# AE-HYU/monte_carlo_localization

Measured on AMD Instinct MI355X. Metric: MCL updates/sec (particle*beam/s), higher is better.
Workload: dtype f64; 1 GPU; 4194304 particles/GPU x 1081 beams, Spielberg_map (2000x2000 @ 0.05796), initial cloud N((0.0, 0.0, 0.0),(0.5 m,0.5 m,0.4 rad)) (tracking regime), action (0.05, 0.0, 0.01), stock sensor/motion params, multinomial resampling, Philox seed 42; the timed updates follow 5 warm-up updates (the particle set has resampled to motion-noise width); particles_total=4194304, beams=1081, parallelism=single GPU

## Files before the change

monte_carlo_localization_amd/csrc/mcl_engine.hip:

```cpp
#include "../../include/mcl_hip_engine.h"

#include <hip/hip_runtime.h>
#include <hip/hip_ext.h>
#include <rocprim/device/device_radix_sort.hpp>

#include <algorithm>
#include <chrono>
#include <cmath>
#include <cstdio>
#include <cstring>
#include <string>
#include <vector>

#include "mcl_engine_internal.h"
#include "mcl_kernels.h"
#include "mcl_host_math.h"
#include "mcl_lfield.h"

static_assert(MCL_WEDGES == mcl::kWedges || MCL_KWEDGES != 16, "include/mcl_hip_engine.h and csrc/mcl_wedge.h disagree");

using namespace mcl_host;

namespace {

thread_local std::string g_create_error;

int ensure_lt(mcl_engine *h)
{
    size_t need = (size_t)(h->P + 1) * h->bpad;
    if (need > h->lt_capacity) {
        dfree(h->d_Lt);
        HIPCHK(h, hipMalloc(&h->d_Lt, 2 * need * sizeof(float)));
        h->lt_capacity = need;
    }
    h->ltd_cols = (h->B + 2 * h->beam_margin + 64) & ~63;
    const size_t need_d = (size_t)mcl::sweep_table_rows(h->P) * h->ltd_cols;
    if (need_d > h->ltd_capacity) {
        dfree(h->d_Ltd);
        HIPCHK(h, hipMalloc(&h->d_Ltd, need_d * sizeof(double)));
        h->ltd_capacity = need_d;
        h->ltd_ready = false;
    }
    return MCL_OK;
}

void build_ltd(mcl_engine *h);

int weight_stats(mcl_engine *h, bool from_log, const double *d_max_override, bool defer_sums = false)
{
    const int64_t n = h->N;
    const double *src = from_log ? h->d_logw : h->d_w;
    const double *max_parts = nullptr;
    if (!d_max_override) {
        if (!(from_log && h->max_partials_ready))
            hipLaunchKernelGGL(mcl::k_reduce_max, dim3(mcl::kRedBlocks), dim3(mcl::kRedThreads), 0, h->stream, src, n, h->d_maxpart);
        max_parts = h->d_maxpart;
    }
    h->max_partials_ready = false;
    hipLaunchKernelGGL(mcl::k_weights, dim3(mcl::kRedBlocks), dim3(mcl::kRedThreads), 0, h->stream, src, from_log ? 1 : 0,
                       d_max_override ? d_max_override : h->d_scalars, h->d_x[h->cur], h->d_y[h->cur], h->d_th[h->cur], n, h->d_w, h->d_q, h->d_part,
                       (from_log && h->cfg.resample_neff_permille > 0) ? h->d_carry[h->carry_idx ^ 1] : (double *)nullptr,
                       max_parts, mcl::kRedBlocks);
    h->carry_pending = from_log && h->cfg.resample_neff_permille > 0;
    if (!from_log) h->carry_valid = false;
    if (defer_sums) h->sums_pending = true;
    else hipLaunchKernelGGL(mcl::k_final_sums, dim3(1), dim3(mcl::kRedThreads), 0, h->stream, h->d_part, mcl::kRedBlocks, h->d_scalars);
    HIPCHK(h, hipGetLastError());
    return MCL_OK;
}

int fetch_scalars(mcl_engine *h)
{
    HIPCHK(h, hipMemcpyAsync(h->h_result, h->d_result, kResultWords * 8, hipMemcpyDeviceToHost, h->stream));
    HIPCHK(h, hipStreamSynchronize(h->stream));
    unpack_result(h);
    return MCL_OK;
}

bool sweep_hybrid(const mcl_engine *h)
{
    return h->sweep_global && h->env_sweep_hybrid != 0 && h->rec_ok && h->sweep_hyb_layout_ok && h->d_beam_err != nullptr &&
           h->d_distw != nullptr && h->d_distg != nullptr && (size_t)mcl::kSwWinBytes + (size_t)h->ltd_cols * 8 <= 80 * 1024 - 64;
}

bool sweep_far_expected(const mcl_engine *h) { return h->far_fresh || h->h_result[15] >= mcl::kFarWindowedMin / 2; }
bool sweep_hybrid_decide(mcl_engine *h)
{
    if (!sweep_hybrid(h)) return false;
    if (h->env_sweep_hybrid == 2) return true;
    if (h->far_fresh) { h->hyb_backoff = 0; h->hyb_skip = 0; return false; }
    if (h->last_sweep_global == 2) {
        if (h->h_result[15] >= mcl::kFarWindowedMin / 2) { h->hyb_backoff = h->hyb_backoff ? std::min(32, 2 * h->hyb_backoff) : 1; h->hyb_skip = h->hyb_backoff; }
        else h->hyb_backoff = 0;
    }
    if (h->hyb_skip > 0) { --h->hyb_skip; return false; }
// ... 586 lines not shown
}

int mcl_host::fail(mcl_engine *h, int code, const char *msg) { if (h) h->err = msg; return code; }
int mcl_host::fail(mcl_engine *h, int code, const std::string &msg) { return fail(h, code, msg.c_str()); }

std::string &mcl_host::create_error() { return g_create_error; }

bool mcl_host::ready(mcl_engine *h, bool need_particles)
{
    return h && h->have_map && h->B > 0 && (!need_particles || h->have_particles);
}

float mcl_host::elapsed(hipEvent_t a, hipEvent_t b)
{
    float ms = 0.f;
    (void)hipEventElapsedTime(&ms, a, b);
    return ms;
}

void mcl_host::graph_reset(mcl_engine *h)
{
    for (int k = 0; k < 2; ++k)
        if (h->graph_exec[k]) { (void)hipGraphExecDestroy(h->graph_exec[k]); h->graph_exec[k] = nullptr; }
    h->graph_warm = false;
    h->prep_cache_valid = false; h->prep_folded = false;
    h->layout_valid = false; h->layout_stale_used = false; h->keys_done = false;
    h->pc_ready = false;
}

int mcl_host::scan_weights(mcl_engine *h, const uint64_t *d_q, uint64_t *d_cdf, int64_t n, uint64_t offset, uint64_t *d_total)
{
    int nb = (int)((n + mcl::kScanTile - 1) / mcl::kScanTile);
    mcl::CompactOut co{};
    const bool own = d_q == h->d_q && d_cdf == h->d_cdf && offset == 0 && !h->env_no_compact && h->d_ccdf;
    if (own) {
        co.block_cnt = h->d_blockcnt; co.ccdf = h->d_ccdf; co.cidx = h->d_cidx; co.crec = h->d_crec; co.ctop = h->d_ctop;
        co.x = h->d_x[h->cur]; co.y = h->d_y[h->cur]; co.th = h->d_th[h->cur];
        co.cap = (uint32_t)h->compact_cap; co.total = h->d_result + 16;
    }
    hipLaunchKernelGGL(mcl::k_scan_partials, dim3(nb), dim3(mcl::kScanThreads), 0, h->stream, d_q, n, h->d_blocktot, co.block_cnt);
    const bool fold = h->sums_pending && d_q == h->d_q;
    hipLaunchKernelGGL(mcl::k_scan_spine, dim3(1), dim3(1024), 0, h->stream, h->d_blocktot, nb, offset, d_total, co.block_cnt, co.total,
                       fold ? h->d_part : (const double *)nullptr, mcl::kRedBlocks, h->d_scalars);
    if (fold) h->sums_pending = false;
    const size_t nlead = (size_t)((n + 15) >> mcl::kLeaderShift) + 1;
    if (nlead > h->leaders_capacity) {
        graph_reset(h);
        dfree(h->d_leaders);
        HIPCHK(h, hipMalloc(&h->d_leaders, nlead * 8));
        h->leaders_capacity = nlead;
    }
    if (h->bind_sensor_event && own && !h->capturing) {
        hipExtLaunchKernelGGL(mcl::k_scan_final, dim3(nb), dim3(mcl::kScanThreads), 0, h->stream, nullptr, h->ev[EV_SENSOR], 0, d_q, n, h->d_blocktot, d_cdf,
                              h->d_leaders, co);
        h->ev_sensor_bound = true; h->bind_sensor_event = false;
    } else {
        hipLaunchKernelGGL(mcl::k_scan_final, dim3(nb), dim3(mcl::kScanThreads), 0, h->stream, d_q, n, h->d_blocktot, d_cdf, h->d_leaders, co);
    }
    HIPCHK(h, hipGetLastError());
    h->blocktot_for = d_cdf; h->blocktot_n = n;
    if (d_cdf == h->d_cdf) { h->compact_n = -1; h->compact_pending = own; h->list_epoch++; }
    return MCL_OK;
}

void mcl_host::unpack_result(mcl_engine *h)
{
    std::memcpy(h->h_scalars, h->h_result, 8 * sizeof(double));
    std::memcpy(h->h_counters, h->h_result + 8, 4 * sizeof(unsigned long long));
    h->h_fix_count = h->h_result[12];
    uint64_t qt;
    std::memcpy(&qt, &h->h_scalars[2], 8);
    h->q_total = qt;
    h->global_sums[0] = h->h_scalars[1];
    h->global_sums[1] = h->h_scalars[3];
    h->global_sums[2] = h->h_scalars[4];
    h->global_sums[3] = h->h_scalars[5];
    h->global_sums[4] = h->h_scalars[6];
    if (h->compact_pending) {
        const unsigned long long na = h->h_result[16];
        h->compact_n = na <= (unsigned long long)h->compact_cap ? (int64_t)na : -1;
        h->compact_pending = false;
    }
}

int mcl_abi_version(void) { return MCL_ABI_VERSION; }

const char *mcl_last_error(const mcl_engine_t *h) { return h ? h->err.c_str() : g_create_error.c_str(); }

int mcl_create(const mcl_config_t *cfg, mcl_engine_t **out)
{
// ... 11 lines not shown
    }
    if (const char *why = bad_sensor_fields(*cfg)) { g_create_error = why; return MCL_ERR_INVALID_ARG; }
    {
        const double disp[3] = {cfg->motion_dispersion_x, cfg->motion_dispersion_y, cfg->motion_dispersion_theta};
        for (double v : disp)
            if (!std::isfinite(v) || v < 0.0) {
                g_create_error = "bad config (motion_dispersion_x/y/theta must be finite and >= 0)";
                return MCL_ERR_INVALID_ARG;
            }
    }
    int ndev = 0;
    if (hipGetDeviceCount(&ndev) != hipSuccess || ndev <= 0 || cfg->device < 0 || cfg->device >= ndev) {
        g_create_error = "no HIP device (this engine has no CPU path)";
        return MCL_ERR_NO_DEVICE;
    }
    hipDeviceProp_t prop;
    if (hipSetDevice(cfg->device) != hipSuccess || hipGetDeviceProperties(&prop, cfg->device) != hipSuccess) {
        g_create_error = "hipSetDevice/hipGetDeviceProperties failed";
        return MCL_ERR_NO_DEVICE;
    }
    if (std::strncmp(prop.gcnArchName, "gfx950", 6) != 0) {
        g_create_error = std::string("device is ") + prop.gcnArchName + ", engine is built for gfx950 only";
        return MCL_ERR_NO_DEVICE;
    }
    mcl_engine *h = new mcl_engine();
    h->cfg = *cfg;
    if (const char *e = getenv("MCL_CELL_MIN")) h->env_cell_min = atoll(e);
    if (const char *e = getenv("MCL_CELL_SLICE")) h->env_cell_slice = atoll(e);
    if (const char *e = getenv("MCL_QSLICES_PER_CU")) h->env_qslices_per_cu = atoi(e);
    if (const char *e = getenv("MCL_QSIDE")) h->env_qside = atoi(e);
    if (const char *e = getenv("MCL_SWEEP_G")) h->env_sweep_g = atoi(e);
    if (const char *e = getenv("MCL_TINY_POLL")) h->env_tiny_poll = atoi(e);
    if (const char *e = getenv("MCL_NO_COMPACT")) h->env_no_compact = atoi(e);
    if (const char *e = getenv("MCL_SORT")) h->env_sort_radix = std::strcmp(e, "radix") == 0 ? 1 : (std::strcmp(e, "hist") == 0 ? 0 : -1);
    if (const char *e = getenv("MCL_DEBUG_WG")) h->env_debug_wg = e;
    h->env_no_bucket_cuts = getenv("MCL_NO_BUCKET_CUTS") != nullptr;
    if (const char *e = getenv("MCL_SWEEP_GLOBAL")) h->env_sweep_global = atoi(e) != 0;
    if (const char *e = getenv("MCL_SWEEP_HYBRID")) h->env_sweep_hybrid = atoi(e);
    if (const char *e = getenv("MCL_SW_GUIDE")) h->env_sw_guide = atoi(e);
    if (const char *e = getenv("MCL_SW_SPLIT16")) h->env_sw_split16 = atoi(e) != 0;
    if (const char *e = getenv("MCL_SWEEP_PAIRS")) h->env_sweep_pairs = atoi(e) != 0 ? 1 : 0;
    h->env_no_obs_overlap = getenv("MCL_NO_OBS_OVERLAP") != nullptr;
    h->env_no_prep_fold = getenv("MCL_NO_PREP_FOLD") != nullptr;
    h->env_no_stale_layout = getenv("MCL_NO_STALE_LAYOUT") != nullptr;
    h->env_comm_no_pregather = getenv("MCL_COMM_NO_PREGATHER") != nullptr;
    h->env_comm_no_lists = getenv("MCL_COMM_NO_LISTS") != nullptr;
    h->num_cu = prop.multiProcessorCount;
    h->cap = cfg->max_particles;
    auto bail = [&](const char *what) {
        g_create_error = std::string(what) + ": " + h->err;
        mcl_destroy(h);
        return MCL_ERR_HIP;
    };
#define CRT(call)                                                         \
    do {                                                                  \
        hipError_t e_ = (call);                                           \
        if (e_ != hipSuccess) { h->err = hipGetErrorString(e_); return bail(#call); } \
    } while (0)
    CRT(hipStreamCreateWithFlags(&h->stream, hipStreamNonBlocking));
    CRT(hipStreamCreateWithFlags(&h->stream2, hipStreamNonBlocking));
    CRT(hipEventCreateWithFlags(&h->ev_obs, hipEventDisableTiming));
    for (int i = 0; i < EV_COUNT; ++i) CRT(hipEventCreate(&h->ev[i]));
    const size_t nb = (size_t)h->cap * sizeof(double);
    for (int b = 0; b < 2; ++b) {
        CRT(hipMalloc(&h->d_x[b], nb)); CRT(hipMalloc(&h->d_y[b], nb)); CRT(hipMalloc(&h->d_th[b], nb));
        CRT(hipMalloc(&h->d_pack[b], (size_t)h->cap * sizeof(double4)));
    }
    CRT(hipMalloc(&h->d_w, nb)); CRT(hipMalloc(&h->d_logw, nb)); CRT(hipMalloc(&h->d_tmp, nb * 3));
    CRT(hipMalloc(&h->d_logw_acc, nb));
    CRT(hipMalloc(&h->d_carry[0], nb)); CRT(hipMalloc(&h->d_carry[1], nb));
    CRT(hipMalloc(&h->d_q, (size_t)h->cap * 8)); CRT(hipMalloc(&h->d_cdf, (size_t)h->cap * 8));
    h->blocktot_capacity = (size_t)h->cap / mcl::kScanTile + 2;
    CRT(hipMalloc(&h->d_blocktot, h->blocktot_capacity * 8));
    CRT(hipMalloc(&h->d_blockcnt, h->blocktot_capacity * 4));
    h->compact_cap = std::max<int64_t>(4096, ((h->cap / 4 + 63) / 64) * 64);
    CRT(hipMalloc(&h->d_ccdf, (size_t)h->compact_cap * 8));
    CRT(hipMalloc(&h->d_ctop, ((size_t)h->compact_cap / 64 + 1) * 8));
    CRT(hipMalloc(&h->d_cidx, (size_t)h->compact_cap * 4));
    CRT(hipMalloc(&h->d_crec, (size_t)h->compact_cap * sizeof(double4)));
    CRT(hipMalloc(&h->d_idx, (size_t)h->cap * 4));
    CRT(hipMalloc(&h->d_part, (size_t)mcl::kRedBlocks * 8 * sizeof(double)));
    CRT(hipMalloc(&h->d_maxpart, (size_t)mcl::kRedBlocks * sizeof(double)));
    CRT(hipMalloc(&h->d_result, 32 * 8));
    CRT(hipMemset(h->d_result, 0, 32 * 8));
    CRT(hipHostMalloc(&h->h_result, 48 * 8));
    std::memset(h->h_result, 0, 48 * 8);
    h->d_scalars = reinterpret_cast<double *>(h->d_result);
    h->d_counters = h->d_result + 8;
    h->d_fix_over = h->d_result + 12;
    CRT(hipMalloc(&h->d_exact_list, (size_t)kExactCap * 8));
    CRT(hipMalloc(&h->d_inject, nb * 4));
    CRT(hipMalloc(&h->d_pc, (size_t)h->cap * sizeof(double4)));
    CRT(hipMalloc(&h->d_qr, (size_t)h->cap * sizeof(short4)));
    CRT(hipMalloc(&h->d_far, (size_t)h->cap * 4));
    CRT(hipMalloc(&h->d_pcs, (size_t)h->cap * sizeof(double4)));
    CRT(hipMalloc(&h->d_ths, (size_t)h->cap * sizeof(double)));
    CRT(hipMalloc(&h->d_perm, (size_t)h->cap * 4));
    CRT(hipMalloc(&h->d_skey, (size_t)h->cap * 4));
    CRT(hipMalloc(&h->d_srank, (size_t)h->cap * 4));
    CRT(hipMalloc(&h->d_hist, (size_t)mcl::kSortBuckets * 4));
    CRT(hipMalloc(&h->d_histpart, (size_t)(mcl::kSortKeySpace / mcl::kHistTile) * 4));
    CRT(hipMalloc(&h->d_tile_used, (size_t)(mcl::kSortKeySpace / mcl::kHistTile) * 4));
    CRT(hipMemset(h->d_hist, 0, (size_t)mcl::kSortBuckets * 4));
    CRT(hipMemset(h->d_tile_used, 0, (size_t)(mcl::kSortKeySpace / mcl::kHistTile) * 4));
    CRT(hipMalloc(&h->d_bbox, 8 * sizeof(int)));
    CRT(hipMalloc(&h->d_bbox_nx, 8 * sizeof(int)));
    CRT(hipMalloc(&h->d_tilemap_nx, (size_t)mcl::kSortMaxTiles * sizeof(int)));
// ... 56 lines not shown
                                     static_lds_is(reinterpret_cast<const void *>(&mcl::k_rays_sweep<true, false, true>), qb) &&
                                     static_lds_is(reinterpret_cast<const void *>(&mcl::k_rays_sweep<false, false, true, true>), qb) &&
                                     static_lds_is(reinterpret_cast<const void *>(&mcl::k_rays_sweep<true, false, true, true>), qb) &&
                                     static_lds_fits(reinterpret_cast<const void *>(&mcl::k_rays_sweep<false, true, true, true>), 0, qb) &&
                                     static_lds_fits(reinterpret_cast<const void *>(&mcl::k_rays_sweep<true, true, true, true>), 0, qb);
        }
#ifdef MCL_LEGACY_RAY_KERNELS
        h->cell_layout_ok = static_lds_is(reinterpret_cast<const void *>(&mcl::k_rays_cell<false>), qb) && static_lds_is(reinterpret_cast<const void *>(&mcl::k_rays_cell<true>), qb);
        h->quad_layout_ok = static_lds_is(reinterpret_cast<const void *>(&mcl::k_rays_quad<false>), qb) && static_lds_is(reinterpret_cast<const void *>(&mcl::k_rays_quad<true>), qb);
#endif
        h->skip_layout_ok = static_lds_is(reinterpret_cast<const void *>(&mcl::k_rays_skip<1, false>), 0) && static_lds_is(reinterpret_cast<const void *>(&mcl::k_rays_skip<1, true>), 0) &&
                            static_lds_is(reinterpret_cast<const void *>(&mcl::k_rays_skip<1, false, true>), 0) && static_lds_is(reinterpret_cast<const void *>(&mcl::k_rays_skip<1, true, true>), 0) &&
                            static_lds_is(reinterpret_cast<const void *>(&mcl::k_rays_skip<2, false>), 0) && static_lds_is(reinterpret_cast<const void *>(&mcl::k_rays_skip<3, false>), 0) &&
                            static_lds_is(reinterpret_cast<const void *>(&mcl::k_rays_skip<4, false>), 0);
        (void)hipGetLastError();
    }
#undef CRT
    *out = h;
    return MCL_OK;
}

void mcl_destroy(mcl_engine_t *h)
{
    if (!h) return;
    (void)hipSetDevice(h->cfg.device);
    if (h->stream) (void)hipStreamSynchronize(h->stream);
    if (h->comm) { comm_free(h->comm); h->comm = nullptr; }
    if (h->clu) { cluster_free(h->clu); h->clu = nullptr; }
    graph_reset(h);
    for (int b = 0; b < 2; ++b) { dfree(h->d_x[b]); dfree(h->d_y[b]); dfree(h->d_th[b]); }
    dfree(h->d_w); dfree(h->d_logw); dfree(h->d_tmp); dfree(h->d_logw_acc); dfree(h->d_carry[0]); dfree(h->d_carry[1]); dfree(h->d_q); dfree(h->d_cdf); dfree(h->d_blocktot); dfree(h->d_bm); dfree(h->d_bm_pop); dfree(h->d_bm_pref);
    dfree(h->d_gcdf); dfree(h->d_gtop);
    dfree(h->d_kld_bm); dfree(h->d_kld_list); dfree(h->d_kld_cnt); dfree(h->d_recov_cnt);
    dfree(h->d_blockcnt); dfree(h->d_ccdf); dfree(h->d_ctop); dfree(h->d_cidx); dfree(h->d_crec);
    dfree(h->d_idx); dfree(h->d_steps); dfree(h->d_part); dfree(h->d_maxpart); dfree(h->d_result); if (h->h_result) { (void)hipHostFree(h->h_result); h->h_result = nullptr; } dfree(h->d_inject); dfree(h->d_pc); dfree(h->d_qr); dfree(h->d_far); dfree(h->d_far_list); dfree(h->d_far_sorted); dfree(h->d_far_cnt); dfree(h->d_pcs); dfree(h->d_ths); dfree(h->d_distw); dfree(h->d_distg); dfree(h->d_leaders); dfree(h->d_pack[0]); dfree(h->d_pack[1]); dfree(h->d_perm); dfree(h->d_skey); dfree(h->d_srank); dfree(h->d_skey2); dfree(h->d_sval2); dfree(h->d_sort_tmp); dfree(h->d_hist); dfree(h->d_histpart); dfree(h->d_tile_used); dfree(h->d_bbox); dfree(h->d_cut_start); dfree(h->d_cut_end); dfree(h->d_tilemap); dfree(h->d_tilemark); dfree(h->d_slice_mean); dfree(h->d_fix_list); dfree(h->d_fix_count); dfree(h->d_exact_list);
    dfree(h->d_grid); dfree(h->d_dist); dfree(h->d_dist4); dfree(h->d_L); dfree(h->d_table);
    dfree(h->d_lf_D); dfree(h->d_lf_tab); dfree(h->d_lf_beams);
    if (h->h_lf_beams) (void)hipHostFree(h->h_lf_beams);
    for (int q = 0; q < 4; ++q) dfree(h->d_distq[q]);
    dfree(h->d_angle); dfree(h->d_beam_cs); dfree(h->d_beam_csx); dfree(h->d_beam_csxg); dfree(h->d_beam_csi); dfree(h->d_beam_err); dfree(h->d_obs_idx); dfree(h->d_Lt); dfree(h->d_Ltd); dfree(h->d_items); dfree(h->d_centres); dfree(h->d_nitems); dfree(h->d_unit_sums); dfree(h->d_unit_begin); dfree(h->d_nunits); dfree(h->d_obs); dfree(h->d_free);
    if (h->h_obs) (void)hipHostFree(h->h_obs);
    for (int i = 0; i < EV_COUNT; ++i)
        if (h->ev[i]) (void)hipEventDestroy(h->ev[i]);
    if (h->ev_obs) (void)hipEventDestroy(h->ev_obs);
    if (h->ev_children) (void)hipEventDestroy(h->ev_children);
    if (h->ev_layout) (void)hipEventDestroy(h->ev_layout);
    if (h->ev_ext_in) (void)hipEventDestroy(h->ev_ext_in);
    if (h->ev_ext_out) (void)hipEventDestroy(h->ev_ext_out);
    dfree(h->d_bbox_nx); dfree(h->d_tilemap_nx); dfree(h->d_tilemark_nx);
    if (h->stream2) { (void)hipStreamSynchronize(h->stream2); (void)hipStreamDestroy(h->stream2); }
    if (h->stream) (void)hipStreamDestroy(h->stream);
    delete h;
}

int mcl_set_map(mcl_engine_t *h, const int8_t *data, uint32_t width, uint32_t height, float resolution, double origin_x,
                double origin_y)
{
    if (!h) return MCL_ERR_INVALID_ARG;
    if (!data || width == 0 || height == 0 || width > 200000 || height > 200000) return fail(h, MCL_ERR_INVALID_ARG, "bad map dimensions");
    int64_t kld_nx = 0, kld_ny = 0;
    uint64_t kld_bits = 0;
    if (h->kld_on && resolution > 0.0f && !kld_grid(&h->kld, width, height, resolution, kld_nx, kld_ny, kld_bits))
        return fail(h, MCL_ERR_INVALID_ARG, "KLD: the bin grid over this map exceeds 2^31 bits");
    if (h->lf_on && resolution > 0.0f && lf_cap(&h->lf, resolution) < 0)
        return fail(h, MCL_ERR_INVALID_ARG, "likelihood field: K = ceil((max_occ_dist_m / resolution)^2) exceeds 65535 on this map");
    graph_reset(h);
    if (!(resolution > 0.0f)) return fail(h, MCL_ERR_INVALID_ARG, "invalid map resolution");
// ... 1715 lines not shown
```

monte_carlo_localization_amd/csrc/mcl_engine_internal.h:

```cpp
#pragma once
#include "../../include/mcl_hip_engine.h"

#include <hip/hip_runtime.h>
#include <hip/hip_ext.h>

#include <cstdint>
#include <string>
#include <vector>

#include "mcl_types.h"
#include "mcl_host_math.h"

enum { EV_START = 0, EV_RESAMPLE, EV_QUERY, EV_RAYS, EV_SENSOR, EV_K0, EV_K1, EV_COUNT };


constexpr unsigned long long kExactCap = 1ull << 16;
constexpr int kResultWords = 18;
constexpr int kResultStage = 40;
constexpr int kResultStamp = 32;
constexpr int kCompactEntryBytes = 44;

struct mcl_comm;
void comm_free(struct mcl_comm *c);
void comm_forget(struct mcl_comm *c);
// ... 89 lines not shown
    bool carry_valid = false, carry_pending = false;
    bool resampled_last = true;
    hipGraphExec_t graph_exec[2] = {nullptr, nullptr};
    bool graph_warm = false;
    bool capturing = false;
    double *d_logw_acc = nullptr;
    uint64_t *d_q = nullptr, *d_cdf = nullptr, *d_blocktot = nullptr;
    uint32_t *d_bm = nullptr;
    uint64_t *d_bm_pop = nullptr, *d_bm_pref = nullptr;
    size_t bm_capacity = 0;
    uint32_t *d_blockcnt = nullptr;
    uint64_t *d_ccdf = nullptr, *d_ctop = nullptr;
    uint32_t *d_cidx = nullptr;
    double4 *d_crec = nullptr;
    int64_t compact_cap = 0;
    int64_t compact_n = -1;
    bool compact_pending = false;
    bool compact_used = false;
    uint64_t *d_gcdf = nullptr, *d_gtop = nullptr;
    size_t gcdf_capacity = 0;
    int env_no_compact = 0;
    uint64_t *d_leaders = nullptr;
    size_t leaders_capacity = 0;
    double4 *d_pack[2]{};
    bool pack_valid[2] = {false, false};
    int32_t *d_idx = nullptr;
    uint8_t *d_steps = nullptr;
    size_t steps_capacity = 0, blocktot_capacity = 0;
    const uint64_t *blocktot_for = nullptr;
    int64_t blocktot_n = 0;
    double *d_part = nullptr;
    double *d_maxpart = nullptr;
    bool sums_pending = false;
    double *d_scalars = nullptr;
    unsigned long long *d_counters = nullptr;
    double *d_inject = nullptr;
    double4 *d_pc = nullptr;
    short4 *d_qr = nullptr;
    bool quad_ok = false;
    int qside = 0;
    unsigned long long *d_fix_list = nullptr, *d_fix_count = nullptr, *d_fix_over = nullptr;
    unsigned long long *d_exact_list = nullptr;
    unsigned long long fix_cap = 0, fix_alloc = 0;
    size_t fix_count_alloc = 0;
    int fix_segments = 0;
    uint8_t *d_far = nullptr;
    uint32_t *d_far_list = nullptr;
    uint32_t *d_far_sorted = nullptr, *d_far_cnt = nullptr;
    double4 *d_pcs = nullptr;
    double *d_ths = nullptr;
    uint8_t *d_distw = nullptr;
    uint32_t *d_perm = nullptr, *d_skey = nullptr, *d_srank = nullptr;
    uint32_t *d_skey2 = nullptr, *d_sval2 = nullptr;
    void *d_sort_tmp = nullptr;
    size_t sort_tmp_bytes = 0;
    int env_sort_radix = -1;
    uint32_t *d_tile_used = nullptr;
    uint32_t *d_hist = nullptr, *d_histpart = nullptr;
    int *d_bbox = nullptr;
    uint32_t *d_cut_start = nullptr, *d_cut_end = nullptr;
    bool env_no_bucket_cuts = false;
    int *d_tilemap = nullptr, *d_tilemark = nullptr;
    int *d_bbox_nx = nullptr, *d_tilemap_nx = nullptr, *d_tilemark_nx = nullptr;
    hipEvent_t ev_children = nullptr, ev_layout = nullptr;
    hipEvent_t ev_ext_in = nullptr, ev_ext_out = nullptr;
    bool stage_async_rays = false, stage_async_weights = false;
// ... 127 lines not shown
```

monte_carlo_localization_amd/csrc/mcl_kernels.h:

```cpp
#pragma once
#include "mcl_types.h"
#include <type_traits>
#include "mcl_device_math.h"
#include "mcl_wedge.h"
#include "mcl_motion.h"

namespace mcl {

constexpr int kRedBlocks = 1024;
constexpr int kRedThreads = 256;
__device__ __forceinline__ void final_sums_of(const double *__restrict__ part, int nb, double *__restrict__ scalars, double (*sm)[7]);


__device__ __forceinline__ uint64_t wave_incl_scan_u64(uint64_t v, int lane)
{
#pragma unroll
    for (int o = 1; o < 64; o <<= 1) {
        uint64_t t = (uint64_t)__shfl_up((long long)v, o, 64);
        if (lane >= o) v += t;
    }
    return v;
}

struct CompactOut {
    uint32_t *block_cnt;
    uint64_t *ccdf;
    uint32_t *cidx;
    double4 *crec;
    uint64_t *ctop;
    const double *x, *y, *th;
    uint32_t cap;
    unsigned long long *total;
};
constexpr int kCompactGroupShift = 6;

__global__ __launch_bounds__(kScanThreads) void k_scan_partials(const uint64_t *__restrict__ q, int64_t n,
                                                               uint64_t *__restrict__ block_tot, uint32_t *__restrict__ block_cnt)
{
    __shared__ uint64_t sm[kScanThreads / 64];
    __shared__ uint32_t smc[kScanThreads / 64];
    int64_t base = (int64_t)blockIdx.x * kScanTile + (int64_t)threadIdx.x * kScanItems;
    uint64_t s = 0;
    uint32_t c = 0;
#pragma unroll
    for (int k = 0; k < kScanItems; ++k)
        if (base + k < n) { const uint64_t v = q[base + k]; s += v; c += v != 0ull; }
    s = wave_sum_u64(s);
    int lane = threadIdx.x & 63, w = threadIdx.x >> 6;
    if (block_cnt) {
#pragma unroll
        for (int o = 32; o > 0; o >>= 1) c += __shfl_xor(c, o, 64);
    }
    if (lane == 0) { sm[w] = s; smc[w] = c; }
    __syncthreads();
    if (threadIdx.x == 0) {
        uint64_t t = 0;
        uint32_t tc = 0;
        for (int i = 0; i < kScanThreads / 64; ++i) { t += sm[i]; tc += smc[i]; }
        block_tot[blockIdx.x] = t;
        if (block_cnt) block_cnt[blockIdx.x] = tc;
    }
}

__global__ __launch_bounds__(1024) void k_scan_spine(uint64_t *__restrict__ block_tot, int nb, uint64_t offset,
                                                     uint64_t *__restrict__ grand_total, uint32_t *__restrict__ block_cnt,
                                                     unsigned long long *__restrict__ alive_total,
                                                     const double *__restrict__ sum_part = nullptr, int n_sum_part = 0, double *__restrict__ scalars = nullptr)
// ... 9 lines not shown
    int lane = threadIdx.x & 63, w = threadIdx.x >> 6;
    if (threadIdx.x == 0) { carry_s = offset; carry_c = 0u; }
    __syncthreads();
    for (int base = 0; base < nb; base += 1024) {
        int i = base + threadIdx.x;
        uint64_t v = (i < nb) ? block_tot[i] : 0;
        uint32_t vc = (block_cnt && i < nb) ? block_cnt[i] : 0u;
        uint64_t inc = wave_incl_scan_u64(v, lane);
        uint32_t incc = vc;
#pragma unroll
        for (int o = 1; o < 64; o <<= 1) { const uint32_t t = __shfl_up(incc, o, 64); if (lane >= o) incc += t; }
        if (lane == 63) { sm[w] = inc; smc[w] = incc; }
        __syncthreads();
        uint64_t woff = 0;
        uint32_t woffc = 0;
        for (int k = 0; k < w; ++k) { woff += sm[k]; woffc += smc[k]; }
        uint64_t carry = carry_s;
        uint32_t carryc = carry_c;
        if (i < nb) {
            block_tot[i] = carry + woff + inc - v;
            if (block_cnt) block_cnt[i] = carryc + woffc + incc - vc;
        }
        __syncthreads();
        if (threadIdx.x == 1023) { carry_s = carry + woff + inc; carry_c = carryc + woffc + incc; }
        __syncthreads();
    }
    if (threadIdx.x == 0 && grand_total) *grand_total = carry_s;
    if (threadIdx.x == 0 && alive_total) *alive_total = (unsigned long long)carry_c;
}

constexpr int kLeaderShift = 4;
__global__ __launch_bounds__(kScanThreads) void k_scan_final(const uint64_t *__restrict__ q, int64_t n,
                                                            const uint64_t *__restrict__ block_off,
                                                            uint64_t *__restrict__ cdf, uint64_t *__restrict__ leaders, CompactOut co)
{
    __shared__ uint64_t sm[kScanThreads / 64];
    __shared__ uint32_t smc[kScanThreads / 64];
    int64_t base = (int64_t)blockIdx.x * kScanTile + (int64_t)threadIdx.x * kScanItems;
    uint64_t v[kScanItems];
    uint64_t s = 0;
    uint32_t alive = 0;
#pragma unroll
    for (int k = 0; k < kScanItems; ++k) {
        uint64_t x = (base + k < n) ? q[base + k] : 0;
        s += x;
        v[k] = s;
        alive |= (x != 0ull ? 1u : 0u) << k;
    }
    int lane = threadIdx.x & 63, w = threadIdx.x >> 6;
    uint64_t inc = wave_incl_scan_u64(s, lane);
    const uint32_t cnt = (uint32_t)__popc(alive);
    uint32_t incc = cnt;
    if (co.block_cnt) {
#pragma unroll
        for (int o = 1; o < 64; o <<= 1) { const uint32_t t = __shfl_up(incc, o, 64); if (lane >= o) incc += t; }
    }
    if (lane == 63) { sm[w] = inc; smc[w] = incc; }
    __syncthreads();
    uint64_t off = block_off[blockIdx.x] + inc - s;
    for (int k = 0; k < w; ++k) off += sm[k];
#pragma unroll
    for (int k = 0; k < kScanItems; ++k)
        if (base + k < n) cdf[base + k] = off + v[k];
    if (leaders) {
        static_assert(kScanItems == 8 && (1 << kLeaderShift) == 16, "a leader is the last item of every second thread");
        const int64_t last = base + kScanItems - 1;
        if ((last & 15) == 15 && last < n) leaders[last >> kLeaderShift] = off + v[kScanItems - 1];
        else if (base < n && n - 1 <= last && ((n - 1) & 15) != 15) leaders[(n - 1) >> kLeaderShift] = off + v[(n - 1) - base];
    }
    if (co.block_cnt && alive) {
        uint32_t pos = co.block_cnt[blockIdx.x] + incc - cnt;
        for (int k = 0; k < w; ++k) pos += smc[k];
#pragma unroll
        for (int k = 0; k < kScanItems; ++k)
            if ((alive >> k) & 1u) {
                if (pos < co.cap) {
                    const int64_t i = base + k;
                    const uint64_t c = off + v[k];
                    co.ccdf[pos] = c;
                    co.cidx[pos] = (uint32_t)i;
                    co.crec[pos] = make_double4(co.x[i], co.y[i], co.th[i], 0.0);
                    if ((pos & ((1u << kCompactGroupShift) - 1u)) == (1u << kCompactGroupShift) - 1u) co.ctop[pos >> kCompactGroupShift] = c;
                }
                ++pos;
            }
    }
}


#ifndef MCL_SORT_SUB
#define MCL_SORT_SUB 1
#endif
constexpr int kSortSub = MCL_SORT_SUB;
__device__ __forceinline__ int cell_of(double g, int hi);
__device__ __forceinline__ uint32_t sort_key(const int *__restrict__ bbox, const int *__restrict__ tilemap, int ntx_abs, int cx, int cy, double th,
                                         int64_t n, double fx = 0.0, double fy = 0.0);

__device__ __forceinline__ void prep_small_clear(const PrepClear &clr, int i, int nthreads)
{
    if (clr.fix_count) for (int k = i; k < clr.fix_words; k += nthreads) clr.fix_count[k] = 0ull;
    if (clr.fix_over && i < 2) clr.fix_over[i] = 0ull;
    if (clr.exact_count && i == 0) clr.exact_count[0] = 0ull;
    if (clr.far_count && i == 0) clr.far_count[0] = 0ull;
    if (clr.bbox && i < 7) clr.bbox[i] = i < 2 ? 0x7fffffff : (i < 4 ? (int)0x80000000 : (i == 6 ? clr.bbox_play : 0));
// ... 1741 lines not shown
}

__global__ void k_group_max(GroupMaxArgs a)
{
    double m = -INFINITY;
    for (int i = 0; i < a.n; ++i) m = fmax(m, a.src[i][0]);
    a.out[0] = m;
}

__global__ void k_stage_pack(const unsigned long long *__restrict__ res, double *__restrict__ vec, int n_shards, int self, int listed,
                             unsigned long long list_cap)
{
    const int len = 5 + 3 * n_shards + 2;
    const double *sc = reinterpret_cast<const double *>(res);
    for (int i = threadIdx.x; i < len; i += blockDim.x) {
        double v = 0.0;
        if (i == 0) v = sc[1];
        else if (i < 5) v = sc[2 + i];
        else if (i == 5 + 3 * self) v = (listed && res[16] <= list_cap) ? (double)(res[16] + 1ull) : 0.0;
        else if (i == 6 + 3 * self) v = (double)(res[2] & 0xFFFFFFFFull);
        else if (i == 7 + 3 * self) v = (double)(res[2] >> 32);
        else if (i == len - 2) v = res[12] != 0ull ? 1.0 : 0.0;
        else if (i == len - 1) v = sc[7];
        vec[i] = v;
    }
}

__global__ __launch_bounds__(kRedThreads) void k_weights(const double *__restrict__ logw_or_w, int from_log,
                                                        const double *__restrict__ maxp, const double *__restrict__ x,
                                                        const double *__restrict__ y, const double *__restrict__ th, int64_t n,
                                                        double *__restrict__ w_out, uint64_t *__restrict__ q_out,
                                                        double *__restrict__ part ,
                                                        double *__restrict__ carry_out ,
                                                        const double *__restrict__ max_parts = nullptr, int n_max_parts = 0)
{
    __shared__ double sm[kRedThreads / 64][7];
    double mx;
    if (max_parts) {
        __shared__ double mxs[kRedThreads / 64];
        double m = -INFINITY;
        for (int i = threadIdx.x; i < n_max_parts; i += kRedThreads) m = fmax(m, max_parts[i]);
        m = wave_max(m);
        if ((threadIdx.x & 63) == 0) mxs[threadIdx.x >> 6] = m;
        __syncthreads();
        mx = mxs[0];
        for (int k = 1; k < kRedThreads / 64; ++k) mx = fmax(mx, mxs[k]);
        if (blockIdx.x == 0 && threadIdx.x == 0) const_cast<double *>(maxp)[0] = mx;
    } else {
        mx = *maxp;
    }
    double sw = 0, swx = 0, swy = 0, sws = 0, swc = 0, sww = 0;
    uint64_t sq = 0;
    for (int64_t i = (int64_t)blockIdx.x * kRedThreads + threadIdx.x; i < n; i += (int64_t)gridDim.x * kRedThreads) {
        double w, wq;
        if (from_log) {
            const double lw = logw_or_w[i];
            const double d = lw == -INFINITY ? -INFINITY : lw - mx;
            w = det_exp(d); wq = w; if (carry_out) carry_out[i] = d;
        }
        else {
            w = logw_or_w[i];
            wq = (mx > 0.0 && w > 0.0) ? (w / mx) : 0.0;
        }
        uint64_t q = (uint64_t)(wq * kWeightScale);
        w_out[i] = w;
        q_out[i] = q;
        double s, c;
        sincos(th[i], &s, &c);
        sw += w; sq += q; swx += w * x[i]; swy += w * y[i]; sws += w * s; swc += w * c; sww += w * w;
    }
    sw = wave_sum(sw); swx = wave_sum(swx); swy = wave_sum(swy); sws = wave_sum(sws); swc = wave_sum(swc); sww = wave_sum(sww);
    sq = wave_sum_u64(sq);
    int wv = threadIdx.x >> 6;
    if ((threadIdx.x & 63) == 0) {
        sm[wv][0] = sw; sm[wv][1] = __longlong_as_double((long long)sq); sm[wv][2] = swx; sm[wv][3] = swy; sm[wv][4] = sws; sm[wv][5] = swc; sm[wv][6] = sww;
    }
    __syncthreads();
    if (threadIdx.x == 0) {
        uint64_t tq = 0;
        double t[7] = {0, 0, 0, 0, 0, 0, 0};
        for (int k = 0; k < kRedThreads / 64; ++k) {
            t[0] += sm[k][0]; tq += (uint64_t)__double_as_longlong(sm[k][1]);
            t[2] += sm[k][2]; t[3] += sm[k][3]; t[4] += sm[k][4]; t[5] += sm[k][5]; t[6] += sm[k][6];
        }
        double *p = part + (size_t)blockIdx.x * 8;
        p[0] = t[0]; p[1] = __longlong_as_double((long long)tq); p[2] = t[2]; p[3] = t[3]; p[4] = t[4]; p[5] = t[5]; p[6] = t[6];
    }
}
__device__ __forceinline__ void final_sums_of(const double *__restrict__ part, int nb, double *__restrict__ scalars, double (*sm)[7])
{
    const bool mine = threadIdx.x < kRedThreads;
    double t[7] = {0, 0, 0, 0, 0, 0, 0};
    uint64_t tq = 0;
    if (mine)
        for (int i = threadIdx.x; i < nb; i += kRedThreads) {
            const double *p = part + (size_t)i * 8;
            t[0] += p[0]; tq += (uint64_t)__double_as_longlong(p[1]); t[2] += p[2]; t[3] += p[3]; t[4] += p[4]; t[5] += p[5]; t[6] += p[6];
        }
    t[0] = wave_sum(t[0]); t[2] = wave_sum(t[2]); t[3] = wave_sum(t[3]); t[4] = wave_sum(t[4]); t[5] = wave_sum(t[5]); t[6] = wave_sum(t[6]);
    tq = wave_sum_u64(tq);
    int wv = threadIdx.x >> 6;
    if (mine && (threadIdx.x & 63) == 0) {
// ... 159 lines not shown
```

Measured before the change: 876.6 billion particle*beam/s.

## Fold scan tile partials into weights kernel and drop scan_partials/spine launches

The weights kernel now accumulates per-scan-tile quantized weight sums and alive counts with wave-level atomics. The final scan kernel then derives each tile's offset by summing preceding tile sums directly, instead of running separate partials and spine kernels. A ticket counter lets the last block clear the tile buffers, and block 0 folds the deferred final sums. This removes two kernel launches and a pass over q. The cost is atomics in the weights loop and an O(nb) prefix loop per scan block, which grows quadratically with tile count.

```diff
diff --git a/monte_carlo_localization_amd/csrc/mcl_engine.hip b/monte_carlo_localization_amd/csrc/mcl_engine.hip
--- a/monte_carlo_localization_amd/csrc/mcl_engine.hip
+++ b/monte_carlo_localization_amd/csrc/mcl_engine.hip
@@ -46,6 +46,16 @@
 
 void build_ltd(mcl_engine *h);
 
+bool compact_wanted(const mcl_engine *h) { return !h->env_no_compact && h->d_ccdf; }
+
+void drop_tile_sums(mcl_engine *h)
+{
+    if (!h->scan_prefix_tiles) return;
+    (void)hipMemsetAsync(h->d_tilesum, 0, (size_t)h->scan_prefix_tiles * 8, h->stream);
+    (void)hipMemsetAsync(h->d_tilecnt, 0, (size_t)h->scan_prefix_tiles * 4, h->stream);
+    h->scan_prefix_tiles = 0;
+}
+
 int weight_stats(mcl_engine *h, bool from_log, const double *d_max_override, bool defer_sums = false)
 {
     const int64_t n = h->N;
@@ -57,10 +67,18 @@
         max_parts = h->d_maxpart;
     }
     h->max_partials_ready = false;
+    mcl::ScanEmit se{};
+    drop_tile_sums(h);
+    if (defer_sums && h->env_tail_fold && n > 0) {
+        se.nb = (int)((n + mcl::kScanTile - 1) / mcl::kScanTile);
+        se.tile_sum = h->d_tilesum;
+        se.tile_cnt = compact_wanted(h) ? h->d_tilecnt : (uint32_t *)nullptr;
+        h->scan_prefix_tiles = se.nb; h->scan_prefix_counts = se.tile_cnt != nullptr;
+    }
     hipLaunchKernelGGL(mcl::k_weights, dim3(mcl::kRedBlocks), dim3(mcl::kRedThreads), 0, h->stream, src, from_log ? 1 : 0,
                        d_max_override ? d_max_override : h->d_scalars, h->d_x[h->cur], h->d_y[h->cur], h->d_th[h->cur], n, h->d_w, h->d_q, h->d_part,
                        (from_log && h->cfg.resample_neff_permille > 0) ? h->d_carry[h->carry_idx ^ 1] : (double *)nullptr,
-                       max_parts, mcl::kRedBlocks);
+                       max_parts, mcl::kRedBlocks, se);
     h->carry_pending = from_log && h->cfg.resample_neff_permille > 0;
     if (!from_log) h->carry_valid = false;
     if (defer_sums) h->sums_pending = true;
@@ -713,17 +731,26 @@
 {
     int nb = (int)((n + mcl::kScanTile - 1) / mcl::kScanTile);
     mcl::CompactOut co{};
-    const bool own = d_q == h->d_q && d_cdf == h->d_cdf && offset == 0 && !h->env_no_compact && h->d_ccdf;
+    const bool own = d_q == h->d_q && d_cdf == h->d_cdf && offset == 0 && compact_wanted(h);
     if (own) {
         co.block_cnt = h->d_blockcnt; co.ccdf = h->d_ccdf; co.cidx = h->d_cidx; co.crec = h->d_crec; co.ctop = h->d_ctop;
         co.x = h->d_x[h->cur]; co.y = h->d_y[h->cur]; co.th = h->d_th[h->cur];
         co.cap = (uint32_t)h->compact_cap; co.total = h->d_result + 16;
     }
-    hipLaunchKernelGGL(mcl::k_scan_partials, dim3(nb), dim3(mcl::kScanThreads), 0, h->stream, d_q, n, h->d_blocktot, co.block_cnt);
-    const bool fold = h->sums_pending && d_q == h->d_q;
-    hipLaunchKernelGGL(mcl::k_scan_spine, dim3(1), dim3(1024), 0, h->stream, h->d_blocktot, nb, offset, d_total, co.block_cnt, co.total,
-                       fold ? h->d_part : (const double *)nullptr, mcl::kRedBlocks, h->d_scalars);
-    if (fold) h->sums_pending = false;
+    const bool ready = h->scan_prefix_tiles == nb && d_q == h->d_q && offset == 0 && !d_total && h->scan_prefix_counts == own;
+    mcl::ScanEmit se{};
+    if (ready) {
+        se.nb = nb; se.tile_sum = h->d_tilesum; se.tile_cnt = h->d_tilecnt; se.ticket = h->d_ticket; se.block_off = h->d_blocktot;
+        if (h->sums_pending) { se.part = h->d_part; se.n_part = mcl::kRedBlocks; se.scalars = h->d_scalars; h->sums_pending = false; }
+        h->scan_prefix_tiles = 0;
+    } else {
+        drop_tile_sums(h);
+        hipLaunchKernelGGL(mcl::k_scan_partials, dim3(nb), dim3(mcl::kScanThreads), 0, h->stream, d_q, n, h->d_blocktot, co.block_cnt);
+        const bool fold = h->sums_pending && d_q == h->d_q;
+        hipLaunchKernelGGL(mcl::k_scan_spine, dim3(1), dim3(1024), 0, h->stream, h->d_blocktot, nb, offset, d_total, co.block_cnt, co.total,
+                           fold ? h->d_part : (const double *)nullptr, mcl::kRedBlocks, h->d_scalars);
+        if (fold) h->sums_pending = false;
+    }
     const size_t nlead = (size_t)((n + 15) >> mcl::kLeaderShift) + 1;
     if (nlead > h->leaders_capacity) {
         graph_reset(h);
@@ -733,10 +760,10 @@
     }
     if (h->bind_sensor_event && own && !h->capturing) {
         hipExtLaunchKernelGGL(mcl::k_scan_final, dim3(nb), dim3(mcl::kScanThreads), 0, h->stream, nullptr, h->ev[EV_SENSOR], 0, d_q, n, h->d_blocktot, d_cdf,
-                              h->d_leaders, co);
+                              h->d_leaders, co, se);
         h->ev_sensor_bound = true; h->bind_sensor_event = false;
     } else {
-        hipLaunchKernelGGL(mcl::k_scan_final, dim3(nb), dim3(mcl::kScanThreads), 0, h->stream, d_q, n, h->d_blocktot, d_cdf, h->d_leaders, co);
+        hipLaunchKernelGGL(mcl::k_scan_final, dim3(nb), dim3(mcl::kScanThreads), 0, h->stream, d_q, n, h->d_blocktot, d_cdf, h->d_leaders, co, se);
     }
     HIPCHK(h, hipGetLastError());
     h->blocktot_for = d_cdf; h->blocktot_n = n;
@@ -814,6 +841,7 @@
     if (const char *e = getenv("MCL_SWEEP_G")) h->env_sweep_g = atoi(e);
     if (const char *e = getenv("MCL_TINY_POLL")) h->env_tiny_poll = atoi(e);
     if (const char *e = getenv("MCL_NO_COMPACT")) h->env_no_compact = atoi(e);
+    if (const char *e = getenv("MCL_TAIL_FOLD")) h->env_tail_fold = atoi(e);
     if (const char *e = getenv("MCL_SORT")) h->env_sort_radix = std::strcmp(e, "radix") == 0 ? 1 : (std::strcmp(e, "hist") == 0 ? 0 : -1);
     if (const char *e = getenv("MCL_DEBUG_WG")) h->env_debug_wg = e;
     h->env_no_bucket_cuts = getenv("MCL_NO_BUCKET_CUTS") != nullptr;
@@ -855,6 +883,9 @@
     h->blocktot_capacity = (size_t)h->cap / mcl::kScanTile + 2;
     CRT(hipMalloc(&h->d_blocktot, h->blocktot_capacity * 8));
     CRT(hipMalloc(&h->d_blockcnt, h->blocktot_capacity * 4));
+    CRT(hipMalloc(&h->d_tilesum, h->blocktot_capacity * 8)); CRT(hipMemset(h->d_tilesum, 0, h->blocktot_capacity * 8));
+    CRT(hipMalloc(&h->d_tilecnt, h->blocktot_capacity * 4)); CRT(hipMemset(h->d_tilecnt, 0, h->blocktot_capacity * 4));
+    CRT(hipMalloc(&h->d_ticket, sizeof(unsigned int))); CRT(hipMemset(h->d_ticket, 0, sizeof(unsigned int)));
     h->compact_cap = std::max<int64_t>(4096, ((h->cap / 4 + 63) / 64) * 64);
     CRT(hipMalloc(&h->d_ccdf, (size_t)h->compact_cap * 8));
     CRT(hipMalloc(&h->d_ctop, ((size_t)h->compact_cap / 64 + 1) * 8));
@@ -977,7 +1008,7 @@
     dfree(h->d_w); dfree(h->d_logw); dfree(h->d_tmp); dfree(h->d_logw_acc); dfree(h->d_carry[0]); dfree(h->d_carry[1]); dfree(h->d_q); dfree(h->d_cdf); dfree(h->d_blocktot); dfree(h->d_bm); dfree(h->d_bm_pop); dfree(h->d_bm_pref);
     dfree(h->d_gcdf); dfree(h->d_gtop);
     dfree(h->d_kld_bm); dfree(h->d_kld_list); dfree(h->d_kld_cnt); dfree(h->d_recov_cnt);
-    dfree(h->d_blockcnt); dfree(h->d_ccdf); dfree(h->d_ctop); dfree(h->d_cidx); dfree(h->d_crec);
+    dfree(h->d_blockcnt); dfree(h->d_tilesum); dfree(h->d_tilecnt); dfree(h->d_ticket); dfree(h->d_ccdf); dfree(h->d_ctop); dfree(h->d_cidx); dfree(h->d_crec);
     dfree(h->d_idx); dfree(h->d_steps); dfree(h->d_part); dfree(h->d_maxpart); dfree(h->d_result); if (h->h_result) { (void)hipHostFree(h->h_result); h->h_result = nullptr; } dfree(h->d_inject); dfree(h->d_pc); dfree(h->d_qr); dfree(h->d_far); dfree(h->d_far_list); dfree(h->d_far_sorted); dfree(h->d_far_cnt); dfree(h->d_pcs); dfree(h->d_ths); dfree(h->d_distw); dfree(h->d_distg); dfree(h->d_leaders); dfree(h->d_pack[0]); dfree(h->d_pack[1]); dfree(h->d_perm); dfree(h->d_skey); dfree(h->d_srank); dfree(h->d_skey2); dfree(h->d_sval2); dfree(h->d_sort_tmp); dfree(h->d_hist); dfree(h->d_histpart); dfree(h->d_tile_used); dfree(h->d_bbox); dfree(h->d_cut_start); dfree(h->d_cut_end); dfree(h->d_tilemap); dfree(h->d_tilemark); dfree(h->d_slice_mean); dfree(h->d_fix_list); dfree(h->d_fix_count); dfree(h->d_exact_list);
     dfree(h->d_grid); dfree(h->d_dist); dfree(h->d_dist4); dfree(h->d_L); dfree(h->d_table);
     dfree(h->d_lf_D); dfree(h->d_lf_tab); dfree(h->d_lf_beams);
diff --git a/monte_carlo_localization_amd/csrc/mcl_engine_internal.h b/monte_carlo_localization_amd/csrc/mcl_engine_internal.h
--- a/monte_carlo_localization_amd/csrc/mcl_engine_internal.h
+++ b/monte_carlo_localization_amd/csrc/mcl_engine_internal.h
@@ -145,6 +145,12 @@
     double *d_part = nullptr;
     double *d_maxpart = nullptr;
     bool sums_pending = false;
+    uint64_t *d_tilesum = nullptr;
+    uint32_t *d_tilecnt = nullptr;
+    unsigned int *d_ticket = nullptr;
+    int env_tail_fold = 1;
+    int scan_prefix_tiles = 0;
+    bool scan_prefix_counts = false;
     double *d_scalars = nullptr;
     unsigned long long *d_counters = nullptr;
     double *d_inject = nullptr;
diff --git a/monte_carlo_localization_amd/csrc/mcl_kernels.h b/monte_carlo_localization_amd/csrc/mcl_kernels.h
--- a/monte_carlo_localization_amd/csrc/mcl_kernels.h
+++ b/monte_carlo_localization_amd/csrc/mcl_kernels.h
@@ -33,6 +33,17 @@
     unsigned long long *total;
 };
 constexpr int kCompactGroupShift = 6;
+
+struct ScanEmit {
+    uint64_t *tile_sum;
+    uint32_t *tile_cnt;
+    unsigned int *ticket;
+    uint64_t *block_off;
+    const double *part;
+    int n_part;
+    double *scalars;
+    int nb;
+};
 
 __global__ __launch_bounds__(kScanThreads) void k_scan_partials(const uint64_t *__restrict__ q, int64_t n,
                                                                uint64_t *__restrict__ block_tot, uint32_t *__restrict__ block_cnt)
@@ -108,10 +119,44 @@
 constexpr int kLeaderShift = 4;
 __global__ __launch_bounds__(kScanThreads) void k_scan_final(const uint64_t *__restrict__ q, int64_t n,
                                                             const uint64_t *__restrict__ block_off,
-                                                            uint64_t *__restrict__ cdf, uint64_t *__restrict__ leaders, CompactOut co)
-{
+                                                            uint64_t *__restrict__ cdf, uint64_t *__restrict__ leaders, CompactOut co,
+                                                            ScanEmit se = ScanEmit{})
+{
+    static_assert(kScanThreads == kRedThreads, "final_sums_of is called by a workgroup of k_scan_final");
     __shared__ uint64_t sm[kScanThreads / 64];
     __shared__ uint32_t smc[kScanThreads / 64];
+    __shared__ unsigned int last_sh;
+    uint64_t tile_off;
+    uint32_t tile_cnt = 0u;
+    if (se.nb) {
+        __shared__ uint64_t smp[kScanThreads / 64];
+        __shared__ uint32_t smpc[kScanThreads / 64];
+        uint64_t ps = 0;
+        uint32_t pc = 0;
+        for (int i = threadIdx.x; i < (int)blockIdx.x; i += kScanThreads) {
+            ps += se.tile_sum[i];
+            if (co.block_cnt) pc += se.tile_cnt[i];
+        }
+        ps = wave_sum_u64(ps);
+#pragma unroll
+        for (int o = 32; o > 0; o >>= 1) pc += __shfl_xor(pc, o, 64);
+        if ((threadIdx.x & 63) == 0) { smp[threadIdx.x >> 6] = ps; smpc[threadIdx.x >> 6] = pc; }
+        __syncthreads();
+        tile_off = 0;
+        for (int k = 0; k < kScanThreads / 64; ++k) { tile_off += smp[k]; tile_cnt += smpc[k]; }
+        if (threadIdx.x == 0) {
+            se.block_off[blockIdx.x] = tile_off;
+            if (co.block_cnt) co.block_cnt[blockIdx.x] = tile_cnt;
+            last_sh = atomicAdd(se.ticket, 1u) == gridDim.x - 1u ? 1u : 0u;
+        }
+        if (se.part && blockIdx.x == 0) {
+            __shared__ double sums_sm[kRedThreads / 64][7];
+            final_sums_of(se.part, se.n_part, se.scalars, sums_sm);
+        }
+    } else {
+        tile_off = block_off[blockIdx.x];
+        if (co.block_cnt) tile_cnt = co.block_cnt[blockIdx.x];
+    }
     int64_t base = (int64_t)blockIdx.x * kScanTile + (int64_t)threadIdx.x * kScanItems;
     uint64_t v[kScanItems];
     uint64_t s = 0;
@@ -133,7 +178,18 @@
     }
     if (lane == 63) { sm[w] = inc; smc[w] = incc; }
     __syncthreads();
-    uint64_t off = block_off[blockIdx.x] + inc - s;
+    if (se.nb) {
+        if (last_sh) {
+            for (int i = threadIdx.x; i < se.nb; i += kScanThreads) { se.tile_sum[i] = 0ull; se.tile_cnt[i] = 0u; }
+            if (threadIdx.x == 0) *se.ticket = 0u;
+        }
+        if (blockIdx.x == gridDim.x - 1 && threadIdx.x == kScanThreads - 1 && co.block_cnt && co.total) {
+            uint32_t t = tile_cnt + incc;
+            for (int k = 0; k < w; ++k) t += smc[k];
+            *co.total = (unsigned long long)t;
+        }
+    }
+    uint64_t off = tile_off + inc - s;
     for (int k = 0; k < w; ++k) off += sm[k];
 #pragma unroll
     for (int k = 0; k < kScanItems; ++k)
@@ -145,7 +201,7 @@
         else if (base < n && n - 1 <= last && ((n - 1) & 15) != 15) leaders[(n - 1) >> kLeaderShift] = off + v[(n - 1) - base];
     }
     if (co.block_cnt && alive) {
-        uint32_t pos = co.block_cnt[blockIdx.x] + incc - cnt;
+        uint32_t pos = tile_cnt + incc - cnt;
         for (int k = 0; k < w; ++k) pos += smc[k];
 #pragma unroll
         for (int k = 0; k < kScanItems; ++k)
@@ -1953,8 +2009,10 @@
                                                         double *__restrict__ w_out, uint64_t *__restrict__ q_out,
                                                         double *__restrict__ part ,
                                                         double *__restrict__ carry_out ,
-                                                        const double *__restrict__ max_parts = nullptr, int n_max_parts = 0)
-{
+                                                        const double *__restrict__ max_parts = nullptr, int n_max_parts = 0,
+                                                        ScanEmit se = ScanEmit{})
+{
+    static_assert(kScanTile % 64 == 0 && kRedThreads % 64 == 0, "the 64 particles of a wave's step lie in one scan tile");
     __shared__ double sm[kRedThreads / 64][7];
     double mx;
     if (max_parts) {
@@ -1972,23 +2030,38 @@
     }
     double sw = 0, swx = 0, swy = 0, sws = 0, swc = 0, sww = 0;
     uint64_t sq = 0;
-    for (int64_t i = (int64_t)blockIdx.x * kRedThreads + threadIdx.x; i < n; i += (int64_t)gridDim.x * kRedThreads) {
-        double w, wq;
-        if (from_log) {
-            const double lw = logw_or_w[i];
-            const double d = lw == -INFINITY ? -INFINITY : lw - mx;
-            w = det_exp(d); wq = w; if (carry_out) carry_out[i] = d;
-        }
-        else {
-            w = logw_or_w[i];
-            wq = (mx > 0.0 && w > 0.0) ? (w / mx) : 0.0;
-        }
-        uint64_t q = (uint64_t)(wq * kWeightScale);
-        w_out[i] = w;
-        q_out[i] = q;
-        double s, c;
-        sincos(th[i], &s, &c);
-        sw += w; sq += q; swx += w * x[i]; swy += w * y[i]; sws += w * s; swc += w * c; sww += w * w;
+    for (int64_t i0 = (int64_t)blockIdx.x * kRedThreads; i0 < n; i0 += (int64_t)gridDim.x * kRedThreads) {
+        const int64_t i = i0 + threadIdx.x;
+        uint64_t q = 0;
+        if (i < n) {
+            double w, wq;
+            if (from_log) {
+                const double lw = logw_or_w[i];
+                const double d = lw == -INFINITY ? -INFINITY : lw - mx;
+                w = det_exp(d); wq = w; if (carry_out) carry_out[i] = d;
+            }
+            else {
+                w = logw_or_w[i];
+                wq = (mx > 0.0 && w > 0.0) ? (w / mx) : 0.0;
+            }
+            q = (uint64_t)(wq * kWeightScale);
+            w_out[i] = w;
+            q_out[i] = q;
+            double s, c;
+            sincos(th[i], &s, &c);
+            sw += w; sq += q; swx += w * x[i]; swy += w * y[i]; sws += w * s; swc += w * c; sww += w * w;
+        }
+        if (se.nb) {
+            const unsigned long long alive = __ballot(q != 0ull);
+            if (alive) {
+                const uint64_t ws = wave_sum_u64(q);
+                if ((threadIdx.x & 63) == 0) {
+                    const int64_t tile = (i0 + (threadIdx.x & ~63)) / kScanTile;
+                    atomicAdd(reinterpret_cast<unsigned long long *>(&se.tile_sum[tile]), (unsigned long long)ws);
+                    if (se.tile_cnt) atomicAdd(&se.tile_cnt[tile], (unsigned int)__popcll(alive));
+                }
+            }
+        }
     }
     sw = wave_sum(sw); swx = wave_sum(swx); swy = wave_sum(swy); sws = wave_sum(sws); swc = wave_sum(swc); sww = wave_sum(sww);
     sq = wave_sum_u64(sq);
```

Result: no change. 876.4 billion particle*beam/s (-0.0%).
